# aletheia-labs/qp-zk-circuits-rm

Hardware: AMD Instinct MI355X
Metric: Wormhole proofs/sec (whole node) (higher is better)
Workload: dtype u64 (Goldilocks field); 1 GPU; batch256_wormhole_proofs_per_gpu; circuit=wormhole deg13 (135 wires), batch_per_gpu=256, provers_per_gpu=3, step_schedule=pipelined, parallelism=proofs sharded x1, RCCL gather of leaf proofs

## Files before the change

### qp-zk-circuits-rm_amd/csrc/ntt16.h

```cpp
#pragma once
#include "field.h"
#include "kernels.h"
#include "field_nc.h"

namespace nt {

using gfn::EPS;
using gfn::canon;
using gfn::mul;
using gfn::sub;

__device__ __forceinline__ uint64_t add_mad(uint64_t a, uint64_t b) {
  uint32_t c0, c1;
  const uint32_t lo = __builtin_addc((uint32_t)a, (uint32_t)b, 0u, &c0);
  const uint32_t hi = __builtin_addc((uint32_t)(a >> 32), (uint32_t)(b >> 32), c0, &c1);
  const uint64_t s = ((uint64_t)hi << 32) | lo;
  const uint32_t e = 0u - c1;
  uint64_t s2, c2, s3, cd;
  uint32_t e2;
  asm("v_mad_u64_u32 %0, %1, %2, 1, %3" : "=v"(s2), "=s"(c2) : "v"(e), "v"(s));
  asm(QP_CWAIT "v_cndmask_b32_e64 %0, 0, -1, %1" : "=v"(e2) : "s"(c2));
  asm("v_mad_u64_u32 %0, %1, %2, 1, %3" : "=v"(s3), "=s"(cd) : "v"(e2), "v"(s2));
  return s3;
}

__device__ __forceinline__ uint64_t add(uint64_t a, uint64_t b) { return add_mad(a, b); }

__device__ __forceinline__ uint64_t reduce(uint64_t lo, uint64_t hi) {
  const uint64_t hh = hi >> 32, hl = hi & EPS;
  uint64_t t0 = lo - hh;
  t0 -= (lo < hh) ? EPS : 0;
  const uint64_t t1 = (hl << 32) - hl;
  const uint64_t r = t0 + t1;
  return r + (r < t1 ? EPS : 0);
}

template <bool K = true, class TW>
__device__ __forceinline__ void mul_rows(uint64_t r[16], const TW &tw) {
  if constexpr (K) {
#pragma unroll
    for (int m = 1; m < 16; m += 3) {
      const uint64_t a[3] = {r[m], r[m + 1], r[m + 2]}, b[3] = {tw(m), tw(m + 1), tw(m + 2)};
      uint64_t o[3];
      gfn::mulk<3>(a, b, o);
      r[m] = o[0];
      r[m + 1] = o[1];
      r[m + 2] = o[2];
    }
  } else {
#pragma unroll
    for (int m = 1; m < 16; m++) r[m] = mul(r[m], tw(m));
  }
}

__device__ __forceinline__ uint64_t neg(uint64_t x) {
  x = canon(x);
  return x ? gl::P - x : 0;
}

__device__ __forceinline__ uint64_t sub_borrow_eps(uint32_t r0, uint32_t r1, uint64_t b) {
  uint32_t e;
  uint64_t c;
  asm(QP_CWAIT "v_cndmask_b32_e64 %0, 0, -1, %1" : "=v"(e) : "s"(b));
  asm("v_sub_co_u32_e64 %0, %1, %2, %3" : "=v"(r0), "=s"(c) : "v"(r0), "v"(e));
  asm(QP_CWAIT "v_subb_co_u32_e64 %0, %1, %2, 0, %3" : "=v"(r1), "=s"(c) : "v"(r1), "s"(c));
  return ((uint64_t)r1 << 32) | r0;
}


template <int E>
__device__ __forceinline__ uint64_t mul_pow2(uint64_t x) {
  if constexpr (E >= 96) {
    return neg(mul_pow2<E - 96>(x));
  } else if constexpr (E == 0) {
    return x;
  } else if constexpr (E >= 32 && E < 64) {
    const uint64_t lo = x << E, hi = x >> (64 - E);
    uint64_t t, c;
    uint32_t e;
    asm("v_mad_u64_u32 %0, %1, %2, -1, %3" : "=v"(t), "=s"(c) : "v"((uint32_t)hi), "v"(lo));
    asm(QP_CWAIT "v_cndmask_b32_e64 %0, 0, -1, %1" : "=v"(e) : "s"(c));
    asm("v_mad_u64_u32 %0, %1, %2, 1, %3" : "=v"(t), "=s"(c) : "v"(e), "v"(t));
    uint32_t r0, r1;
    asm("v_sub_co_u32_e64 %0, %1, %2, %3" : "=v"(r0), "=s"(c) : "v"((uint32_t)t), "v"((uint32_t)(hi >> 32)));
    asm(QP_CWAIT "v_subb_co_u32_e64 %0, %1, %2, 0, %3" : "=v"(r1), "=s"(c) : "v"((uint32_t)(t >> 32)), "s"(c));
    return sub_borrow_eps(r0, r1, c);
  } else if constexpr (E >= 64) {
    constexpr int F = E - 64;
    const uint64_t u = (uint64_t)(uint32_t)x << F, v = (x >> 32) << F;
    const uint64_t S = v + (uint32_t)u + (uint32_t)(u >> 32);
    uint32_t r0, r1;
    uint64_t c;
    asm("v_sub_co_u32_e64 %0, %1, 0, %2" : "=v"(r0), "=s"(c) : "v"((uint32_t)S));
    asm(QP_CWAIT "v_subb_co_u32_e64 %0, %1, %2, %3, %1" : "=v"(r1), "+s"(c) : "v"((uint32_t)u), "v"((uint32_t)(S >> 32)));
    return sub_borrow_eps(r0, r1, c);
  } else {
    return reduce(x << E, x >> (64 - E));
  }
}

template <bool INV, int J>
__device__ __forceinline__ uint64_t mul_w16(uint64_t x) {
  if constexpr (J == 0) return x;
  else if constexpr (!INV) return mul_pow2<(12 * J) % 192>(x);
  else return mul_pow2<(192 - 12 * J) % 192>(x);
}

__device__ __forceinline__ void add4(const uint64_t a[4], const uint64_t b[4], uint64_t s[4]) {
  uint64_t c0, c1, c2, c3;
  uint32_t e0, e1, e2, e3;
  asm("v_lshl_add_u64 %0, %12, 0, %16\n\t"
      "v_lshl_add_u64 %1, %13, 0, %17\n\t"
      "v_lshl_add_u64 %2, %14, 0, %18\n\t"
      "v_lshl_add_u64 %3, %15, 0, %19\n\t"
      "v_cmp_lt_u64_e64 %8, %0, %16\n\t"
      "v_cmp_lt_u64_e64 %9, %1, %17\n\t"
      "v_cmp_lt_u64_e64 %10, %2, %18\n\t"
      "v_cmp_lt_u64_e64 %11, %3, %19\n\t"
      "v_cndmask_b32_e64 %4, 0, -1, %8\n\t"
      "v_cndmask_b32_e64 %5, 0, -1, %9\n\t"
      "v_cndmask_b32_e64 %6, 0, -1, %10\n\t"
      "v_cndmask_b32_e64 %7, 0, -1, %11\n\t"
      "v_mad_u64_u32 %0, %8, %4, 1, %0\n\t"
      "v_mad_u64_u32 %1, %9, %5, 1, %1\n\t"
      "v_mad_u64_u32 %2, %10, %6, 1, %2\n\t"
      "v_mad_u64_u32 %3, %11, %7, 1, %3\n\t"
      "v_cndmask_b32_e64 %4, 0, -1, %8\n\t"
      "v_cndmask_b32_e64 %5, 0, -1, %9\n\t"
      "v_cndmask_b32_e64 %6, 0, -1, %10\n\t"
      "v_cndmask_b32_e64 %7, 0, -1, %11\n\t"
      "v_mad_u64_u32 %0, %8, %4, 1, %0\n\t"
      "v_mad_u64_u32 %1, %9, %5, 1, %1\n\t"
      "v_mad_u64_u32 %2, %10, %6, 1, %2\n\t"
      "v_mad_u64_u32 %3, %11, %7, 1, %3"
      : "=&v"(s[0]), "=&v"(s[1]), "=&v"(s[2]), "=&v"(s[3]), "=&v"(e0), "=&v"(e1), "=&v"(e2), "=&v"(e3),
        "=&s"(c0), "=&s"(c1), "=&s"(c2), "=&s"(c3)
      : "v"(a[0]), "v"(a[1]), "v"(a[2]), "v"(a[3]), "v"(b[0]), "v"(b[1]), "v"(b[2]), "v"(b[3]));
}

__device__ __forceinline__ void sub4(const uint64_t a[4], const uint64_t b[4], uint64_t d[4]) {
  uint32_t l0, l1, l2, l3, h0, h1, h2, h3, e0, e1, e2, e3;
  uint64_t c0, c1, c2, c3;
  asm("v_sub_co_u32_e64 %0, %12, %16, %24\n\t"
      "v_sub_co_u32_e64 %1, %13, %17, %25\n\t"
      "v_sub_co_u32_e64 %2, %14, %18, %26\n\t"
      "v_sub_co_u32_e64 %3, %15, %19, %27\n\t"
      "v_subb_co_u32_e64 %4, %12, %20, %28, %12\n\t"
      "v_subb_co_u32_e64 %5, %13, %21, %29, %13\n\t"
      "v_subb_co_u32_e64 %6, %14, %22, %30, %14\n\t"
      "v_subb_co_u32_e64 %7, %15, %23, %31, %15\n\t"
      "v_cndmask_b32_e64 %8, 0, -1, %12\n\t"
      "v_cndmask_b32_e64 %9, 0, -1, %13\n\t"
      "v_cndmask_b32_e64 %10, 0, -1, %14\n\t"
      "v_cndmask_b32_e64 %11, 0, -1, %15\n\t"
      "v_sub_co_u32_e64 %0, %12, %0, %8\n\t"
      "v_sub_co_u32_e64 %1, %13, %1, %9\n\t"
      "v_sub_co_u32_e64 %2, %14, %2, %10\n\t"
      "v_sub_co_u32_e64 %3, %15, %3, %11\n\t"
      "v_subb_co_u32_e64 %4, %12, %4, 0, %12\n\t"
      "v_subb_co_u32_e64 %5, %13, %5, 0, %13\n\t"
      "v_subb_co_u32_e64 %6, %14, %6, 0, %14\n\t"
      "v_subb_co_u32_e64 %7, %15, %7, 0, %15\n\t"
      "v_cndmask_b32_e64 %8, 0, -1, %12\n\t"
      "v_cndmask_b32_e64 %9, 0, -1, %13\n\t"
      "v_cndmask_b32_e64 %10, 0, -1, %14\n\t"
      "v_cndmask_b32_e64 %11, 0, -1, %15\n\t"
      "v_sub_co_u32_e64 %0, %12, %0, %8\n\t"
      "v_sub_co_u32_e64 %1, %13, %1, %9\n\t"
      "v_sub_co_u32_e64 %2, %14, %2, %10\n\t"
      "v_sub_co_u32_e64 %3, %15, %3, %11\n\t"
      "v_subb_co_u32_e64 %4, %12, %4, 0, %12\n\t"
      "v_subb_co_u32_e64 %5, %13, %5, 0, %13\n\t"
      "v_subb_co_u32_e64 %6, %14, %6, 0, %14\n\t"
      "v_subb_co_u32_e64 %7, %15, %7, 0, %15"
      : "=&v"(l0), "=&v"(l1), "=&v"(l2), "=&v"(l3), "=&v"(h0), "=&v"(h1), "=&v"(h2), "=&v"(h3), "=&v"(e0),
        "=&v"(e1), "=&v"(e2), "=&v"(e3), "=&s"(c0), "=&s"(c1), "=&s"(c2), "=&s"(c3)
      : "v"((uint32_t)a[0]), "v"((uint32_t)a[1]), "v"((uint32_t)a[2]), "v"((uint32_t)a[3]),
        "v"((uint32_t)(a[0] >> 32)), "v"((uint32_t)(a[1] >> 32)), "v"((uint32_t)(a[2] >> 32)),
        "v"((uint32_t)(a[3] >> 32)), "v"((uint32_t)b[0]), "v"((uint32_t)b[1]), "v"((uint32_t)b[2]),
        "v"((uint32_t)b[3]), "v"((uint32_t)(b[0] >> 32)), "v"((uint32_t)(b[1] >> 32)), "v"((uint32_t)(b[2] >> 32)),
        "v"((uint32_t)(b[3] >> 32)));
  d[0] = ((uint64_t)h0 << 32) | l0;
  d[1] = ((uint64_t)h1 << 32) | l1;
  d[2] = ((uint64_t)h2 << 32) | l2;
  d[3] = ((uint64_t)h3 << 32) | l3;
}

template <bool INV, int H>
__device__ __forceinline__ void stage16(uint64_t a[16]) {
#pragma unroll
  for (int g = 0; g < 8; g += 4) {
    int lo[4];
#pragma unroll
    for (int i = 0; i < 4; i++) lo[i] = ((g + i) / H) * 2 * H + (g + i) % H;
    uint64_t u[4], v[4], s[4], d[4];
#pragma unroll
    for (int i = 0; i < 4; i++) {
      u[i] = a[lo[i]];
      v[i] = a[lo[i] + H];
    }
    add4(u, v, s);
    sub4(u, v, d);
#pragma unroll
    for (int i = 0; i < 4; i++) {
      a[lo[i]] = s[i];
      switch ((lo[i] % H) * (8 / H)) {
        case 0: a[lo[i] + H] = d[i]; break;
        case 1: a[lo[i] + H] = mul_w16<INV, 1>(d[i]); break;
        case 2: a[lo[i] + H] = mul_w16<INV, 2>(d[i]); break;
        case 3: a[lo[i] + H] = mul_w16<INV, 3>(d[i]); break;
        case 4: a[lo[i] + H] = mul_w16<INV, 4>(d[i]); break;
        case 5: a[lo[i] + H] = mul_w16<INV, 5>(d[i]); break;
        case 6: a[lo[i] + H] = mul_w16<INV, 6>(d[i]); break;
        default: a[lo[i] + H] = mul_w16<INV, 7>(d[i]); break;
      }
    }
  }
}

template <bool INV>
__device__ __forceinline__ void dft16(uint64_t a[16]) {
  stage16<INV, 8>(a);
  stage16<INV, 4>(a);
  stage16<INV, 2>(a);
  stage16<INV, 1>(a);
}

__device__ __forceinline__ uint64_t tw_pow(const uint64_t *__restrict__ tw, uint32_t e, uint32_t log_S) {
  return qpk::tw_get(tw, e << (qpk::TW_LOG - log_S));
}

__host__ __device__ __forceinline__ constexpr uint32_t lp(uint32_t i) { return i + (i >> 5); }

__device__ __forceinline__ uint32_t brev4(uint32_t m) { return __builtin_bitreverse32(m) >> 28; }

template <bool INV, int H, int S>
__device__ __forceinline__ void stage_small(uint64_t r[S]) {
#pragma unroll
  for (int k = 0; k < S; k += 2 * H) {
#pragma unroll
    for (int j = 0; j < H; j++) {
      const uint64_t u = r[k + j], v = r[k + j + H];
      r[k + j] = add(u, v);
      const uint64_t d = sub(u, v);
      switch (j * (8 / H)) {
        case 0: r[k + j + H] = d; break;
        case 1: r[k + j + H] = mul_w16<INV, 1>(d); break;
        case 2: r[k + j + H] = mul_w16<INV, 2>(d); break;
        case 3: r[k + j + H] = mul_w16<INV, 3>(d); break;
        case 4: r[k + j + H] = mul_w16<INV, 4>(d); break;
        case 5: r[k + j + H] = mul_w16<INV, 5>(d); break;
        case 6: r[k + j + H] = mul_w16<INV, 6>(d); break;
        default: r[k + j + H] = mul_w16<INV, 7>(d); break;
      }
    }
  }
}

template <bool INV, int LOGS>
__device__ __forceinline__ void tail(uint64_t *a, uint32_t n) {
  constexpr int S = 1 << LOGS;
  for (uint32_t g = threadIdx.x; g < (n >> LOGS); g += blockDim.x) {
    uint64_t *base = a + lp(g << LOGS);
    uint64_t r[S];
#pragma unroll
    for (int m = 0; m < S; m++) r[m] = base[m];
    if constexpr (S >= 8) stage_small<INV, S / 2, S>(r);
    if constexpr (S >= 4) stage_small<INV, 2, S>(r);
    stage_small<INV, 1, S>(r);
#pragma unroll
    for (int m = 0; m < S; m++) base[m] = r[m];
  }
  __syncthreads();
}

template <bool INV>
__device__ __forceinline__ uint64_t mul_w32(uint64_t x, int j) {
#define QP_W32(J) \
  case J: return INV ? mul_pow2<(192 - 6 * J) % 192>(x) : mul_pow2<(6 * J) % 192>(x);
  switch (j) {
    QP_W32(1) QP_W32(2) QP_W32(3) QP_W32(4) QP_W32(5) QP_W32(6) QP_W32(7) QP_W32(8)
    QP_W32(9) QP_W32(10) QP_W32(11) QP_W32(12) QP_W32(13) QP_W32(14) QP_W32(15)
    default: return x;
  }
#undef QP_W32
}

template <bool INV>
__device__ __forceinline__ void pass32(uint64_t *a, uint32_t n) {
  for (uint32_t g = threadIdx.x; g < (n >> 4); g += blockDim.x) {
    const uint32_t t = (g >> 6) & 1, sp = ((g >> 7) << 6) | (g & 63);
    uint64_t *base = a + lp((sp << 5) + t);
    uint64_t r[16];
#pragma unroll
    for (int m = 0; m < 16; m++) r[m] = base[lp(2 * m)];
    dft16<INV>(r);
    if (t) {
#pragma unroll
      for (int m = 1; m < 16; m++) r[m] = mul_w32<INV>(r[m], (int)brev4(m));
    }
#pragma unroll
    for (int m = 0; m < 16; m++) base[lp(2 * m)] = r[m];
  }
  __syncthreads();
}

__host__ __device__ constexpr bool use_pass32(uint32_t log_S, uint32_t n, uint32_t T) {
  return log_S == 5 && (n >> 4) % 128 == 0 && T % 64 == 0;
}
__host__ __device__ constexpr uint32_t lds_levels_left(uint32_t log_n, uint32_t log_S, uint32_t T) {
  while (log_S >= 4) log_S = use_pass32(log_S, 1u << log_n, T) ? 1 : log_S - 4;
  return log_S;
}
template <bool INV, bool TAIL = true, bool K = true>
__device__ __forceinline__ uint32_t ntt_lds_from(uint64_t *a, uint32_t log_n, uint32_t log_S, const uint64_t *__restrict__ pt) {
  const uint32_t n = 1u << log_n;
  const uint32_t T = blockDim.x;
  while (log_S >= 4) {
    if (use_pass32(log_S, n, T)) {
      pass32<INV>(a, n);
      log_S = 1;
      continue;
    }
    const uint32_t S = 1u << log_S, q = S >> 4, log_q = log_S - 4;
    for (uint32_t g = threadIdx.x; g < (n >> 4); g += T) {
      const uint32_t sp = g >> log_q, t = g & (q - 1);
      uint64_t *base = a + lp((sp << log_S) + t);
      uint64_t r[16];
#pragma unroll
      for (int m = 0; m < 16; m++) r[m] = base[lp(m * q)];
      dft16<INV>(r);
      if (t) {
        const uint64_t *ptS = pt + qpk::pt_offset(log_S) + t;
        mul_rows<K>(r, [&](int m) { return ptS[m * q]; });
      }
#pragma unroll
      for (int m = 0; m < 16; m++) base[lp(m * q)] = r[m];
    }
    __syncthreads();
    log_S -= 4;
  }
  if (!TAIL) return log_S;
  if (log_S == 1) tail<INV, 1>(a, n);
  else if (log_S == 2) tail<INV, 2>(a, n);
  else if (log_S == 3) tail<INV, 3>(a, n);
  return 0;
}

template <bool INV, int LOGS>
__device__ __forceinline__ void tail_group(uint64_t r[1 << LOGS]) {
  constexpr int S = 1 << LOGS;
  if constexpr (S >= 8) stage_small<INV, S / 2, S>(r);
  if constexpr (S >= 4) stage_small<INV, 2, S>(r);
  if constexpr (S >= 2) stage_small<INV, 1, S>(r);
}

template <bool INV>
__device__ __forceinline__ void ntt_lds(uint64_t *a, uint32_t log_n, const uint64_t *__restrict__ pt) {
  ntt_lds_from<INV, true>(a, log_n, log_n, pt);
}


__device__ __forceinline__ uint32_t brev3(uint32_t m) { return __builtin_bitreverse32(m) >> 29; }

template <bool INV>
__device__ __forceinline__ void dft8(uint64_t a[8]) {
  stage_small<INV, 4, 8>(a);
  stage_small<INV, 2, 8>(a);
  stage_small<INV, 1, 8>(a);
}

template <bool INV>
__device__ __forceinline__ uint64_t mul_w16_rt(uint64_t x, int j) {
#define QP_W16(J) \
  case J: return mul_w16<INV, J>(x);
  switch (j) {
    QP_W16(1) QP_W16(2) QP_W16(3) QP_W16(4) QP_W16(5) QP_W16(6) QP_W16(7)
    default: return x;
  }
#undef QP_W16
}

template <bool INV>
__device__ __forceinline__ void ntt8_lds_from(uint64_t *a, uint32_t log_n, uint32_t log_S,
                                              const uint64_t *__restrict__ tw) {
  const uint32_t n = 1u << log_n;
  const uint32_t T = blockDim.x;
  while (log_S >= 3) {
    if (log_S == 4 && (n >> 3) % 128 == 0 && T % 64 == 0) {
      for (uint32_t g = threadIdx.x; g < (n >> 3); g += T) {
        const uint32_t t = (g >> 6) & 1, sp = ((g >> 7) << 6) | (g & 63);
        uint64_t *base = a + lp((sp << 4) + t);
        uint64_t r[8];
#pragma unroll
        for (int m = 0; m < 8; m++) r[m] = base[lp(2 * m)];
        dft8<INV>(r);
        if (t) {
#pragma unroll
          for (int m = 1; m < 8; m++) r[m] = mul_w16_rt<INV>(r[m], (int)brev3(m));
        }
#pragma unroll
        for (int m = 0; m < 8; m++) base[lp(2 * m)] = r[m];
      }
      __syncthreads();
      log_S = 1;
      break;
    }
    const uint32_t q = 1u << (log_S - 3), log_q = log_S - 3;
    for (uint32_t g = threadIdx.x; g < (n >> 3); g += T) {
      const uint32_t sp = g >> log_q, t = g & (q - 1);
      uint64_t *base = a + lp((sp << log_S) + t);
      uint64_t r[8];
#pragma unroll
      for (int m = 0; m < 8; m++) r[m] = base[lp(m * q)];
      dft8<INV>(r);
      if (t) {
#pragma unroll
        for (int m = 1; m < 8; m++) r[m] = mul(r[m], tw_pow(tw, t * brev3(m), log_S));
      }
#pragma unroll
      for (int m = 0; m < 8; m++) base[lp(m * q)] = r[m];
    }
    __syncthreads();
    log_S -= 3;
  }
  if (log_S == 1) tail<INV, 1>(a, n);
  else if (log_S == 2) tail<INV, 2>(a, n);
}

}
```

Baseline: 1327 proofs/s.

## Use lazy 96-bit redundant representation in radix-16 DFT butterflies

Replaces per-butterfly Goldilocks modular add/sub/twiddle-multiply in dft16 with a three-limb (96-bit) lazy representation. Additions and subtractions keep a signed top word, and twiddle multiplies become shifts by powers of two reduced via shl3. A single fold back to canonical 64-bit happens only at the end, plus a few pre-folds where limbs could overflow. This is meant to cut per-stage reduction instructions, at the cost of more live registers and correctness subtleties in the bounds analysis.

```diff
diff --git a/qp-zk-circuits-rm_amd/csrc/ntt16.h b/qp-zk-circuits-rm_amd/csrc/ntt16.h
--- a/qp-zk-circuits-rm_amd/csrc/ntt16.h
+++ b/qp-zk-circuits-rm_amd/csrc/ntt16.h
@@ -186,33 +186,227 @@
   d[3] = ((uint64_t)h3 << 32) | l3;
 }
 
+struct T3 {
+  uint32_t l0, l1, t;
+};
+__device__ __forceinline__ T3 t3(uint64_t x) { return {(uint32_t)x, (uint32_t)(x >> 32), 0u}; }
+
+template <bool Z>
+__device__ __forceinline__ void add3x4(const T3 a[4], const T3 b[4], T3 s[4]) {
+  uint64_t c0, c1, c2, c3;
+  if constexpr (Z) {
+    asm("v_add_co_u32_e64 %0, %12, %16, %24\n\t"
+        "v_add_co_u32_e64 %1, %13, %17, %25\n\t"
+        "v_add_co_u32_e64 %2, %14, %18, %26\n\t"
+        "v_add_co_u32_e64 %3, %15, %19, %27\n\t"
+        "v_addc_co_u32_e64 %4, %12, %20, %28, %12\n\t"
+        "v_addc_co_u32_e64 %5, %13, %21, %29, %13\n\t"
+        "v_addc_co_u32_e64 %6, %14, %22, %30, %14\n\t"
+        "v_addc_co_u32_e64 %7, %15, %23, %31, %15\n\t"
+        "v_cndmask_b32_e64 %8, 0, 1, %12\n\t"
+        "v_cndmask_b32_e64 %9, 0, 1, %13\n\t"
+        "v_cndmask_b32_e64 %10, 0, 1, %14\n\t"
+        "v_cndmask_b32_e64 %11, 0, 1, %15"
+        : "=&v"(s[0].l0), "=&v"(s[1].l0), "=&v"(s[2].l0), "=&v"(s[3].l0), "=&v"(s[0].l1), "=&v"(s[1].l1),
+          "=&v"(s[2].l1), "=&v"(s[3].l1), "=&v"(s[0].t), "=&v"(s[1].t), "=&v"(s[2].t), "=&v"(s[3].t), "=&s"(c0),
+          "=&s"(c1), "=&s"(c2), "=&s"(c3)
+        : "v"(a[0].l0), "v"(a[1].l0), "v"(a[2].l0), "v"(a[3].l0), "v"(a[0].l1), "v"(a[1].l1), "v"(a[2].l1),
+          "v"(a[3].l1), "v"(b[0].l0), "v"(b[1].l0), "v"(b[2].l0), "v"(b[3].l0), "v"(b[0].l1), "v"(b[1].l1),
+          "v"(b[2].l1), "v"(b[3].l1));
+  } else {
+    asm("v_add_co_u32_e64 %0, %12, %16, %28\n\t"
+        "v_add_co_u32_e64 %1, %13, %17, %29\n\t"
+        "v_add_co_u32_e64 %2, %14, %18, %30\n\t"
+        "v_add_co_u32_e64 %3, %15, %19, %31\n\t"
+        "v_addc_co_u32_e64 %4, %12, %20, %32, %12\n\t"
+        "v_addc_co_u32_e64 %5, %13, %21, %33, %13\n\t"
+        "v_addc_co_u32_e64 %6, %14, %22, %34, %14\n\t"
+        "v_addc_co_u32_e64 %7, %15, %23, %35, %15\n\t"
+        "v_addc_co_u32_e64 %8, %12, %24, %36, %12\n\t"
+        "v_addc_co_u32_e64 %9, %13, %25, %37, %13\n\t"
+        "v_addc_co_u32_e64 %10, %14, %26, %38, %14\n\t"
+        "v_addc_co_u32_e64 %11, %15, %27, %39, %15"
+        : "=&v"(s[0].l0), "=&v"(s[1].l0), "=&v"(s[2].l0), "=&v"(s[3].l0), "=&v"(s[0].l1), "=&v"(s[1].l1),
+          "=&v"(s[2].l1), "=&v"(s[3].l1), "=&v"(s[0].t), "=&v"(s[1].t), "=&v"(s[2].t), "=&v"(s[3].t), "=&s"(c0),
+          "=&s"(c1), "=&s"(c2), "=&s"(c3)
+        : "v"(a[0].l0), "v"(a[1].l0), "v"(a[2].l0), "v"(a[3].l0), "v"(a[0].l1), "v"(a[1].l1), "v"(a[2].l1),
+          "v"(a[3].l1), "v"(a[0].t), "v"(a[1].t), "v"(a[2].t), "v"(a[3].t), "v"(b[0].l0), "v"(b[1].l0),
+          "v"(b[2].l0), "v"(b[3].l0), "v"(b[0].l1), "v"(b[1].l1), "v"(b[2].l1), "v"(b[3].l1), "v"(b[0].t),
+          "v"(b[1].t), "v"(b[2].t), "v"(b[3].t));
+  }
+}
+
+template <bool Z>
+__device__ __forceinline__ void sub3x4(T3 d[4], const T3 b[4]) {
+  uint64_t c0, c1, c2, c3;
+  if constexpr (Z) {
+    asm("v_sub_co_u32_e64 %0, %12, %0, %16\n\t"
+        "v_sub_co_u32_e64 %1, %13, %1, %17\n\t"
+        "v_sub_co_u32_e64 %2, %14, %2, %18\n\t"
+        "v_sub_co_u32_e64 %3, %15, %3, %19\n\t"
+        "v_subb_co_u32_e64 %4, %12, %4, %20, %12\n\t"
+        "v_subb_co_u32_e64 %5, %13, %5, %21, %13\n\t"
+        "v_subb_co_u32_e64 %6, %14, %6, %22, %14\n\t"
+        "v_subb_co_u32_e64 %7, %15, %7, %23, %15\n\t"
+        "v_cndmask_b32_e64 %8, 0, -1, %12\n\t"
+        "v_cndmask_b32_e64 %9, 0, -1, %13\n\t"
+        "v_cndmask_b32_e64 %10, 0, -1, %14\n\t"
+        "v_cndmask_b32_e64 %11, 0, -1, %15"
+        : "+v"(d[0].l0), "+v"(d[1].l0), "+v"(d[2].l0), "+v"(d[3].l0), "+v"(d[0].l1), "+v"(d[1].l1), "+v"(d[2].l1),
+          "+v"(d[3].l1), "=&v"(d[0].t), "=&v"(d[1].t), "=&v"(d[2].t), "=&v"(d[3].t), "=&s"(c0), "=&s"(c1),
+          "=&s"(c2), "=&s"(c3)
+        : "v"(b[0].l0), "v"(b[1].l0), "v"(b[2].l0), "v"(b[3].l0), "v"(b[0].l1), "v"(b[1].l1), "v"(b[2].l1),
+          "v"(b[3].l1));
+  } else {
+    asm("v_sub_co_u32_e64 %0, %12, %0, %16\n\t"
+        "v_sub_co_u32_e64 %1, %13, %1, %17\n\t"
+        "v_sub_co_u32_e64 %2, %14, %2, %18\n\t"
+        "v_sub_co_u32_e64 %3, %15, %3, %19\n\t"
+        "v_subb_co_u32_e64 %4, %12, %4, %20, %12\n\t"
+        "v_subb_co_u32_e64 %5, %13, %5, %21, %13\n\t"
+        "v_subb_co_u32_e64 %6, %14, %6, %22, %14\n\t"
+        "v_subb_co_u32_e64 %7, %15, %7, %23, %15\n\t"
+        "v_subb_co_u32_e64 %8, %12, %8, %24, %12\n\t"
+        "v_subb_co_u32_e64 %9, %13, %9, %25, %13\n\t"
+        "v_subb_co_u32_e64 %10, %14, %10, %26, %14\n\t"
+        "v_subb_co_u32_e64 %11, %15, %11, %27, %15"
+        : "+v"(d[0].l0), "+v"(d[1].l0), "+v"(d[2].l0), "+v"(d[3].l0), "+v"(d[0].l1), "+v"(d[1].l1), "+v"(d[2].l1),
+          "+v"(d[3].l1), "+v"(d[0].t), "+v"(d[1].t), "+v"(d[2].t), "+v"(d[3].t), "=&s"(c0), "=&s"(c1), "=&s"(c2),
+          "=&s"(c3)
+        : "v"(b[0].l0), "v"(b[1].l0), "v"(b[2].l0), "v"(b[3].l0), "v"(b[0].l1), "v"(b[1].l1), "v"(b[2].l1),
+          "v"(b[3].l1), "v"(b[0].t), "v"(b[1].t), "v"(b[2].t), "v"(b[3].t));
+  }
+}
+
+__device__ __forceinline__ uint64_t fold(const T3 x) {
+  const uint64_t l = ((uint64_t)x.l1 << 32) | x.l0;
+  uint64_t r, c;
+  uint32_t e, c1, c2;
+  asm("v_mad_u64_u32 %0, %1, %2, -1, %3" : "=v"(r), "=s"(c) : "v"(x.t), "v"(l));
+  asm(QP_CWAIT "v_cndmask_b32_e64 %0, 0, -1, %1" : "=v"(e) : "s"(c));
+  uint32_t r0 = __builtin_addc((uint32_t)r, e, x.t >> 31, &c1);
+  const uint32_t r1 = __builtin_addc((uint32_t)(r >> 32), 0u, c1, &c2);
+  r0 -= c2;
+  return ((uint64_t)r1 << 32) | r0;
+}
+
+__device__ __forceinline__ void fold4(const T3 x[4], uint64_t o[4]) {
+  uint64_t r[4], c0, c1, c2, c3, s0, s1, s2, s3;
+  uint32_t e0, e1, e2, e3;
+  const uint64_t l[4] = {((uint64_t)x[0].l1 << 32) | x[0].l0, ((uint64_t)x[1].l1 << 32) | x[1].l0,
+                         ((uint64_t)x[2].l1 << 32) | x[2].l0, ((uint64_t)x[3].l1 << 32) | x[3].l0};
+  asm("v_mad_u64_u32 %0, %8, %16, -1, %20\n\t"
+      "v_mad_u64_u32 %1, %9, %17, -1, %21\n\t"
+      "v_mad_u64_u32 %2, %10, %18, -1, %22\n\t"
+      "v_mad_u64_u32 %3, %11, %19, -1, %23\n\t"
+      "v_cmp_gt_i32_e64 %12, 0, %16\n\t"
+      "v_cmp_gt_i32_e64 %13, 0, %17\n\t"
+      "v_cmp_gt_i32_e64 %14, 0, %18\n\t"
+      "v_cmp_gt_i32_e64 %15, 0, %19\n\t"
+      "v_cndmask_b32_e64 %4, 0, -1, %8\n\t"
+      "v_cndmask_b32_e64 %5, 0, -1, %9\n\t"
+      "v_cndmask_b32_e64 %6, 0, -1, %10\n\t"
+      "v_cndmask_b32_e64 %7, 0, -1, %11"
+      : "=&v"(r[0]), "=&v"(r[1]), "=&v"(r[2]), "=&v"(r[3]), "=&v"(e0), "=&v"(e1), "=&v"(e2), "=&v"(e3), "=&s"(c0),
+        "=&s"(c1), "=&s"(c2), "=&s"(c3), "=&s"(s0), "=&s"(s1), "=&s"(s2), "=&s"(s3)
+      : "v"(x[0].t), "v"(x[1].t), "v"(x[2].t), "v"(x[3].t), "v"(l[0]), "v"(l[1]), "v"(l[2]), "v"(l[3]));
+  uint32_t a0 = (uint32_t)r[0], a1 = (uint32_t)r[1], a2 = (uint32_t)r[2], a3 = (uint32_t)r[3];
+  uint32_t b0 = (uint32_t)(r[0] >> 32), b1 = (uint32_t)(r[1] >> 32), b2 = (uint32_t)(r[2] >> 32),
+           b3 = (uint32_t)(r[3] >> 32);
+  asm("v_addc_co_u32_e64 %0, %8, %0, %12, %8\n\t"
+      "v_addc_co_u32_e64 %1, %9, %1, %13, %9\n\t"
+      "v_addc_co_u32_e64 %2, %10, %2, %14, %10\n\t"
+      "v_addc_co_u32_e64 %3, %11, %3, %15, %11\n\t"
+      "v_addc_co_u32_e64 %4, %8, %4, 0, %8\n\t"
+      "v_addc_co_u32_e64 %5, %9, %5, 0, %9\n\t"
+      "v_addc_co_u32_e64 %6, %10, %6, 0, %10\n\t"
+      "v_addc_co_u32_e64 %7, %11, %7, 0, %11\n\t"
+      "v_subb_co_u32_e64 %0, %8, %0, 0, %8\n\t"
+      "v_subb_co_u32_e64 %1, %9, %1, 0, %9\n\t"
+      "v_subb_co_u32_e64 %2, %10, %2, 0, %10\n\t"
+      "v_subb_co_u32_e64 %3, %11, %3, 0, %11"
+      : "+v"(a0), "+v"(a1), "+v"(a2), "+v"(a3), "+v"(b0), "+v"(b1), "+v"(b2), "+v"(b3), "+s"(s0), "+s"(s1), "+s"(s2),
+        "+s"(s3)
+      : "v"(e0), "v"(e1), "v"(e2), "v"(e3));
+  o[0] = ((uint64_t)b0 << 32) | a0;
+  o[1] = ((uint64_t)b1 << 32) | a1;
+  o[2] = ((uint64_t)b2 << 32) | a2;
+  o[3] = ((uint64_t)b3 << 32) | a3;
+}
+
+template <int E>
+__device__ __forceinline__ T3 shl3(const T3 x) {
+  if constexpr (E == 0) {
+    return x;
+  } else if constexpr (E < 32) {
+    return {x.l0 << E, (x.l1 << E) | (x.l0 >> (32 - E)), (x.t << E) | (x.l1 >> (32 - E))};
+  } else if constexpr (E < 64) {
+    constexpr int R = 64 - E;
+    const uint32_t w1 = x.l0 << (E - 32), w2 = (x.l1 << (32 - R)) | (x.l0 >> R);
+    const uint32_t h = (x.t << (32 - R)) | (x.l1 >> R), hs = (uint32_t)((int32_t)h >> 31);
+    uint64_t T, c;
+    uint32_t ce, b0, b1, b2;
+    asm("v_mad_u64_u32 %0, %1, %2, -1, %3" : "=v"(T), "=s"(c) : "v"(w2), "v"((uint64_t)w1 << 32));
+    asm(QP_CWAIT "v_cndmask_b32_e64 %0, 0, 1, %1" : "=v"(ce) : "s"(c));
+    T3 o;
+    o.l0 = __builtin_subc((uint32_t)T, h, 0u, &b0);
+    o.l1 = __builtin_subc((uint32_t)(T >> 32), hs, b0, &b1);
+    o.t = __builtin_subc(ce, hs, b1, &b2);
+    return o;
+  } else {
+    constexpr int F = E - 64, R = 32 - F;
+    const uint32_t w2 = x.l0 << F;
+    const uint32_t z0 = (x.l1 << F) | (x.l0 >> R), z1 = (x.t << F) | (x.l1 >> R);
+    const uint32_t zs = (uint32_t)((int32_t)z1 >> 31);
+    const uint64_t T = (uint64_t)w2 * EPS;
+    uint32_t b0, b1, b2;
+    T3 o;
+    o.l0 = __builtin_subc((uint32_t)T, z0, 0u, &b0);
+    o.l1 = __builtin_subc((uint32_t)(T >> 32), z1, b0, &b1);
+    o.t = __builtin_subc(0u, zs, b1, &b2);
+    return o;
+  }
+}
+
+template <bool INV, int J>
+constexpr int w16_exp = J == 0 ? 0 : INV ? 96 - 12 * J : 12 * J;
+
+template <bool INV>
+__host__ __device__ constexpr bool need_prefold(int H, int idx) {
+  return (H == 4 && (idx == 14 || idx == (INV ? 15 : 13))) || (H == 2 && (idx == 7 || idx == 15));
+}
+
 template <bool INV, int H>
-__device__ __forceinline__ void stage16(uint64_t a[16]) {
+__device__ __forceinline__ void stage16(T3 a[16]) {
 #pragma unroll
   for (int g = 0; g < 8; g += 4) {
     int lo[4];
 #pragma unroll
     for (int i = 0; i < 4; i++) lo[i] = ((g + i) / H) * 2 * H + (g + i) % H;
-    uint64_t u[4], v[4], s[4], d[4];
+    T3 u[4], v[4], q[4], s[4], d[4];
 #pragma unroll
     for (int i = 0; i < 4; i++) {
       u[i] = a[lo[i]];
       v[i] = a[lo[i] + H];
-    }
-    add4(u, v, s);
-    sub4(u, v, d);
+      const bool swap = INV && (lo[i] % H) != 0;
+      d[i] = swap ? v[i] : u[i];
+      q[i] = swap ? u[i] : v[i];
+    }
+    add3x4<H == 8>(u, v, s);
+    sub3x4<H == 8>(d, q);
 #pragma unroll
     for (int i = 0; i < 4; i++) {
       a[lo[i]] = s[i];
+      if (need_prefold<INV>(H, lo[i] + H)) d[i] = t3(fold(d[i]));
       switch ((lo[i] % H) * (8 / H)) {
         case 0: a[lo[i] + H] = d[i]; break;
-        case 1: a[lo[i] + H] = mul_w16<INV, 1>(d[i]); break;
-        case 2: a[lo[i] + H] = mul_w16<INV, 2>(d[i]); break;
-        case 3: a[lo[i] + H] = mul_w16<INV, 3>(d[i]); break;
-        case 4: a[lo[i] + H] = mul_w16<INV, 4>(d[i]); break;
-        case 5: a[lo[i] + H] = mul_w16<INV, 5>(d[i]); break;
-        case 6: a[lo[i] + H] = mul_w16<INV, 6>(d[i]); break;
-        default: a[lo[i] + H] = mul_w16<INV, 7>(d[i]); break;
+        case 1: a[lo[i] + H] = shl3<w16_exp<INV, 1>>(d[i]); break;
+        case 2: a[lo[i] + H] = shl3<w16_exp<INV, 2>>(d[i]); break;
+        case 3: a[lo[i] + H] = shl3<w16_exp<INV, 3>>(d[i]); break;
+        case 4: a[lo[i] + H] = shl3<w16_exp<INV, 4>>(d[i]); break;
+        case 5: a[lo[i] + H] = shl3<w16_exp<INV, 5>>(d[i]); break;
+        case 6: a[lo[i] + H] = shl3<w16_exp<INV, 6>>(d[i]); break;
+        default: a[lo[i] + H] = shl3<w16_exp<INV, 7>>(d[i]); break;
       }
     }
   }
@@ -220,10 +414,16 @@
 
 template <bool INV>
 __device__ __forceinline__ void dft16(uint64_t a[16]) {
-  stage16<INV, 8>(a);
-  stage16<INV, 4>(a);
-  stage16<INV, 2>(a);
-  stage16<INV, 1>(a);
+  T3 x[16];
+#pragma unroll
+  for (int m = 0; m < 16; m++) x[m] = t3(a[m]);
+  stage16<INV, 8>(x);
+  stage16<INV, 4>(x);
+  stage16<INV, 2>(x);
+  stage16<INV, 1>(x);
+#pragma unroll
+  for (int m = 0; m < 16; m++)
+    if (m % 4 == 0) fold4(x + m, a + m);
 }
 
 __device__ __forceinline__ uint64_t tw_pow(const uint64_t *__restrict__ tw, uint32_t e, uint32_t log_S) {
```

After: 1343 proofs/s, median of 6. +1.2%, better.
